# zer0main/npge

Measured on AMD Instinct MI355X. Metric: anchored+aligned Mbp/sec at 1/2/4/8 MI355X; bit-exact anchor set vs CPU, higher is better.
Workload: dtype u8

## Files before the change

### npge_amd/anchor_finder.py

```python
import ctypes

import numpy as np

from . import _capi
from .model import Block, Fragment
from .processor import Decimal, Processor, register


def seqset_for(bs):
    key = tuple((id(s), len(s.data)) for s in bs.seqs)
    cached = getattr(bs, "_npgx_seqset", None)
    if cached is not None and cached[0] == key:
        return cached[1]
    ss = _capi.SeqSet([s.data for s in bs.seqs], [s.name for s in bs.seqs])
    bs._npgx_seqset = (key, ss)
    return ss


@register
class AnchorFinder(Processor):
    name = "AnchorFinder"

    def __init__(self, bloom_params=None):
        super().__init__()
        self.add_gopt("anchor-size", "anchor size", "ANCHOR_SIZE")
        self.add_gopt("anchor-fp", "Probability of false positive in Bloom filter "
                      "(first step of AnchorFinder)", "ANCHOR_FP", Decimal)
        self.add_opt("anchor-similar", "If neighbour anchors are skipped", True)
        self.add_gopt("max-anchor-fragments", "Maximum number of anchors fragments to return",
                      "MAX_ANCHOR_FRAGMENTS")
        self.add_opt("bloom-seed", "glibc srand() seed of the Bloom hash parameters", 1)
        self.add_opt("bloom-epochs", "epochs of the one-GPU Bloom pass (0 = automatic, 1 = single pass)", 0)
        self.add_opt_rule("anchor-size > 0", lambda p: p.opt_value("anchor-size") > 0)
        self.add_opt_rule("anchor-size <= 32", lambda p: p.opt_value("anchor-size") <= 32)
        self.bloom_params = bloom_params
        self._h = None
        self._h_key = None
        self.stats = None

    def _handle(self):
        L = _capi.lib()
        key = (self.opt_value("anchor-size"), self.opt_value("anchor-fp").impl,
               bool(self.opt_value("anchor-similar")), self.opt_value("max-anchor-fragments"),
               self.opt_value("bloom-seed"), tuple(self.bloom_params or ()), self.opt_value("bloom-epochs"))
        if self._h is not None and key == self._h_key:
            return self._h
        if self._h is not None:
            L.npgx_af_free(self._h)
            self._h = None
        o = _capi.AfOptions()
        L.npgx_af_default_options(ctypes.byref(o))
        o.anchor_size, o.anchor_fp_x1e4, o.anchor_similar = key[0], key[1], int(key[2])
        o.max_anchor_fragments, o.bloom_seed = key[3], key[4] & 0xFFFFFFFF
        o.bloom_epochs = key[6]
        if self.bloom_params:
            arr = (ctypes.c_uint64 * len(self.bloom_params))(*self.bloom_params)
            o.n_bloom_params = len(self.bloom_params)
            o.bloom_params = ctypes.cast(arr, ctypes.POINTER(ctypes.c_uint64))
        h = ctypes.c_void_p()
        _capi.check(L.npgx_af_create(ctypes.byref(o), ctypes.byref(h)))
        self._h, self._h_key = h, key
        return h

    def find(self, seqset):
        L = _capi.lib()
        h = self._handle()
        _capi.check(L.npgx_af_run(h, seqset.handle))
        return self.result()

    def find_sharded(self, seqset, comm):
        L = _capi.lib()
        h = self._handle()
        rc = L.npgx_af_run_sharded(h, seqset.handle, comm.pointer())
        if rc != 0 and comm.errors:
            raise _capi.NpgxError(rc, "; ".join(comm.errors))
        _capi.check(rc)
        return self.result()

    def result(self):
        L = _capi.lib()
        h = self._h
        nb, nf = ctypes.c_int64(), ctypes.c_int64()
        _capi.check(L.npgx_af_result_counts(h, ctypes.byref(nb), ctypes.byref(nf)))
        bs = np.zeros(nb.value + 1, dtype=np.int64)
        seq = np.zeros(nf.value, dtype=np.int32)
        mn = np.zeros(nf.value, dtype=np.int64)
        mx = np.zeros(nf.value, dtype=np.int64)
        ori = np.zeros(nf.value, dtype=np.int8)
        _capi.check(L.npgx_af_result_copy(h, _capi.ptr(bs), _capi.ptr(seq), _capi.ptr(mn),
                                          _capi.ptr(mx), _capi.ptr(ori)))
        st = _capi.AfStats()
        _capi.check(L.npgx_af_stats_get(h, ctypes.byref(st)))
        self.stats = st
        return dict(block_start=bs, seq=seq, min_pos=mn, max_pos=mx, ori=ori.astype(np.int32),
                    members=st.members, bits=st.bloom_bits, hashes=st.bloom_hashes,
                    params=np.array(st.bloom_params[:st.bloom_hashes], dtype=np.uint64),
                    n_collected=st.n_collected, n_found_frags=st.n_found_frags,
                    n_windows=st.n_windows)

    def used_hashes(self):
        L = _capi.lib()
        n = ctypes.c_int64()
        _capi.check(L.npgx_af_used_hashes(self._h, None, 0, ctypes.byref(n)))
        out = np.zeros(n.value, dtype=np.uint64)
        _capi.check(L.npgx_af_used_hashes(self._h, _capi.ptr(out), n.value, ctypes.byref(n)))
        return out

    def clear_used(self):
        if self._h is not None:
            _capi.check(_capi.lib().npgx_af_clear_used(self._h))

    def kernel_times(self):
        return _capi.kernel_times(_capi.lib().npgx_af_kernel_times, self._h)

    def run_impl(self):
        bs = self.block_set()
        ss = seqset_for(bs)
        r = self.find(ss)
        b = r["block_start"]
        for i in range(len(b) - 1):
            frs = [Fragment(bs.seqs[int(r["seq"][j])], int(r["min_pos"][j]), int(r["max_pos"][j]),
                            int(r["ori"][j])) for j in range(b[i], b[i + 1])]
            bs.blocks.append(Block(frs))

    def __del__(self):
# ... 7 lines not shown
```

### npge_amd/blockset.py

```python
import ctypes

import numpy as np

from . import _capi


class BbOptions(ctypes.Structure):
    _fields_ = [("extend_length", ctypes.c_int32), ("max_iterations", ctypes.c_int32),
                ("extend_portion_x1e4", ctypes.c_int64), ("min_fragment", ctypes.c_int32),
                ("frame_length", ctypes.c_int32), ("min_end", ctypes.c_int32),
                ("min_block", ctypes.c_int32), ("max_block", ctypes.c_int32),
                ("find_subblocks", ctypes.c_int32), ("min_identity_x1e4", ctypes.c_int64),
                ("align", _capi.AlignOptions), ("max_tail", ctypes.c_int32),
                ("max_tail_to_gap_x1e4", ctypes.c_int64)]


class BbStats(ctypes.Structure):
    _fields_ = [("iterations", ctypes.c_int64), ("aligned_residues", ctypes.c_int64),
                ("align_jobs", ctypes.c_int64), ("anchor_blocks", ctypes.c_int64),
                ("stem_blocks", ctypes.c_int64), ("ms_align", ctypes.c_double),
                ("ms_host", ctypes.c_double), ("ms_stage", ctypes.c_double * 16),
                ("counters", ctypes.c_int64 * 8), ("loop", ctypes.c_int64 * 8),
                ("ms_loop", ctypes.c_double * 8), ("ms_gpu", ctypes.c_double * 12),
                ("device_iterations", ctypes.c_int64), ("device_sync_iterations", ctypes.c_int64)]
# ... 101 lines not shown
            setattr(o.align, k.replace("align_", ""), v)
        else:
            setattr(o, k, v)
    return o


class BlockSetEngine:

    def __init__(self, seqset, options=None, lender=None, **kw):
        L = _bind(_capi.lib())
        self.ss = seqset
        o = options or default_options(**kw)
        h = ctypes.c_void_p()
        if lender is None:
            _capi.check(L.npgx_blockset_create(seqset.handle, ctypes.byref(o), ctypes.byref(h)))
        else:
            _capi.check(L.npgx_blockset_create_sharing(seqset.handle, ctypes.byref(o), lender._h,
                                                       ctypes.byref(h)))
        self._lender = lender
        self._h = h

    def set_comm(self, comm):
        self._comm = comm
        _capi.check(_capi.lib().npgx_blockset_set_comm(self._h, comm.pointer() if comm else None))
        return self

    def set_blocks(self, blocks):
        L = _capi.lib()
        frs = [f for b in blocks for f in b]
        bs = np.zeros(len(blocks) + 1, dtype=np.int64)
        np.cumsum([len(b) for b in blocks], out=bs[1:])
        seq = np.array([f[0] for f in frs] or [0], dtype=np.int32)
        mn = np.array([f[1] for f in frs] or [0], dtype=np.int64)
        mx = np.array([f[2] for f in frs] or [0], dtype=np.int64)
        ori = np.array([f[3] for f in frs] or [1], dtype=np.int8)
        has_rows = any(f[4] is not None for f in frs)
        if has_rows:
            rows = "".join(f[4] or "" for f in frs).encode()
            ro = np.zeros(len(frs) + 1, dtype=np.int64)
            np.cumsum([len(f[4] or "") for f in frs], out=ro[1:])
            buf = ctypes.create_string_buffer(rows, max(len(rows), 1))
            _capi.check(L.npgx_blockset_set_blocks(self._h, len(blocks), _capi.ptr(bs), _capi.ptr(seq),
                                                   _capi.ptr(mn), _capi.ptr(mx), _capi.ptr(ori),
                                                   _capi.ptr(ro), ctypes.cast(buf, ctypes.c_void_p)))
        else:
            _capi.check(L.npgx_blockset_set_blocks(self._h, len(blocks), _capi.ptr(bs), _capi.ptr(seq),
                                                   _capi.ptr(mn), _capi.ptr(mx), _capi.ptr(ori),
                                                   None, None))
        return self

    def apply(self, processor, af=None):
        L = _capi.lib()
        afh = af._handle() if af is not None else None
        _capi.check(L.npgx_blockset_apply(self._h, processor.encode(), afh))
        return self

    def reset_loop(self):
        _capi.check(_capi.lib().npgx_blockset_reset_loop(self._h))
        return self

    def blocks(self):
        L = _capi.lib()
        nb, nf, rb = ctypes.c_int64(), ctypes.c_int64(), ctypes.c_int64()
        _capi.check(L.npgx_blockset_counts(self._h, ctypes.byref(nb), ctypes.byref(nf), ctypes.byref(rb)))
        n = max(nf.value, 1)
        bs = np.zeros(nb.value + 1, dtype=np.int64)
        seq = np.zeros(n, dtype=np.int32)
        mn = np.zeros(n, dtype=np.int64)
        mx = np.zeros(n, dtype=np.int64)
        ori = np.zeros(n, dtype=np.int8)
        ro = np.zeros(n + 1, dtype=np.int64)
        rows = ctypes.create_string_buffer(max(rb.value, 1))
        _capi.check(L.npgx_blockset_copy(self._h, _capi.ptr(bs), _capi.ptr(seq), _capi.ptr(mn),
                                         _capi.ptr(mx), _capi.ptr(ori), _capi.ptr(ro),
                                         ctypes.cast(rows, ctypes.c_void_p)))
        raw = rows.raw
        out = []
        for b in range(nb.value):
            blk = []
            for i in range(bs[b], bs[b + 1]):
                row = raw[ro[i]:ro[i + 1]].decode() if ro[i + 1] > ro[i] else None
                blk.append((int(seq[i]), int(mn[i]), int(mx[i]), int(ori[i]), row))
            out.append(blk)
        return out

    def fragments(self):
        L = _capi.lib()
        nb, nf, rb = ctypes.c_int64(), ctypes.c_int64(), ctypes.c_int64()
        _capi.check(L.npgx_blockset_counts(self._h, ctypes.byref(nb), ctypes.byref(nf), ctypes.byref(rb)))
        n = max(nf.value, 1)
        bs = np.zeros(nb.value + 1, dtype=np.int64)
        seq = np.zeros(n, dtype=np.int32)
        mn = np.zeros(n, dtype=np.int64)
        mx = np.zeros(n, dtype=np.int64)
        ori = np.zeros(n, dtype=np.int8)
        _capi.check(L.npgx_blockset_copy(self._h, _capi.ptr(bs), _capi.ptr(seq), _capi.ptr(mn),
                                         _capi.ptr(mx), _capi.ptr(ori), None, None))
        return bs, seq[:nf.value], mn[:nf.value], mx[:nf.value], ori[:nf.value]

    def conseq(self):
        L = _bind(_capi.lib())
        nb, tot = ctypes.c_int64(), ctypes.c_int64()
        _capi.check(L.npgx_blockset_conseq(self._h, None, None, ctypes.byref(nb), ctypes.byref(tot)))
        buf = ctypes.create_string_buffer(max(tot.value, 1))
        off = np.zeros(nb.value + 1, dtype=np.int64)
        _capi.check(L.npgx_blockset_conseq(self._h, ctypes.cast(buf, ctypes.c_void_p), _capi.ptr(off),
# ... 185 lines not shown
```

### npge_amd/csrc/anchor_finder.hip

```cpp
#include <rocprim/device/device_radix_sort.hpp>
#include <rocprim/device/device_scan.hpp>
#include <rocprim/device/device_select.hpp>

#include <algorithm>
#include <cmath>
#include <cstring>
#include <map>

#include <chrono>

#include "common.hpp"

namespace npgx {

std::string genome_of(const std::string& name);
uint64_t estimate_length(const npgx_seqset* s);
int64_t optimal_bits(uint64_t members, double error_prob);
int optimal_hashes(uint64_t members, uint64_t bits);
void glibc_rand(uint32_t seed, int n, uint64_t* out);

static constexpr int WG = 256;
static constexpr int MAX_KB = 32;
static constexpr int FKB = 4;

// ... 405 lines not shown
            return;
        }
        s = (s + 1) & mask;
    }
}

__global__ __launch_bounds__(WG) void k_ff_count(AfArgs a, TableArgs t, uint32_t* __restrict__ counts) {
    const Chunk c = a.chunks[blockIdx.x];
    const SeqMeta s = a.meta[c.seq];
    const int64_t p = c.pos + threadIdx.x;
    if (p + a.k > s.size) return;
    uint64_t dir;
    if (!load_window(a, s, p, dir)) return;
    const uint64_t rev = revcomp(dir, a.k);
    const uint64_t h = dir < rev ? dir : rev;
    const int64_t idx = table_find(t, h);
    if (idx >= 0) atomicAdd(&counts[idx], 1u);
}

__global__ void k_find_cut(const uint32_t* __restrict__ offsets, const uint32_t* __restrict__ counts,
                           int64_t nH, uint64_t max_frag, uint64_t* __restrict__ out ) {
    if (threadIdx.x != 0 || blockIdx.x != 0) return;
    const uint64_t total = nH ? (uint64_t)offsets[nH - 1] + counts[nH - 1] : 0;
    int64_t lo = 0, hi = nH;
    while (lo < hi) {
        int64_t mid = (lo + hi) >> 1;
        if ((uint64_t)offsets[mid] < max_frag) lo = mid + 1;
        else hi = mid;
    }
    out[0] = (uint64_t)lo;
    out[1] = lo < nH ? (uint64_t)offsets[lo] : total;
    out[2] = total;
}

__global__ __launch_bounds__(WG) void k_ff_scatter(AfArgs a, TableArgs t, const uint64_t* __restrict__ H,
                                                   uint64_t G, const uint32_t* __restrict__ offsets,
                                                   uint32_t* __restrict__ cursor, int key_bits,
                                                   uint64_t* __restrict__ cand) {
    const Chunk c = a.chunks[blockIdx.x];
    const SeqMeta s = a.meta[c.seq];
    const int64_t p = c.pos + threadIdx.x;
    if (p + a.k > s.size) return;
    uint64_t dir;
    if (!load_window(a, s, p, dir)) return;
    const uint64_t rev = revcomp(dir, a.k);
    const uint64_t h = dir < rev ? dir : rev;
    if (h > H[G - 1]) return;
    const int64_t idx = table_find(t, h);
    if (idx < 0) return;
    const uint64_t pos2 = (uint64_t)p + (h == dir ? 0ull : (uint64_t)s.size);
    const uint64_t key2 = 2ull * s.order_off + pos2;
    const uint32_t slot = offsets[idx] + atomicAdd(&cursor[idx], 1u);
    cand[slot] = ((uint64_t)idx << key_bits) | key2;
}

__global__ void k_flip_sign(uint32_t* __restrict__ v, int64_t n) {
    const int64_t i = (int64_t)blockIdx.x * blockDim.x + threadIdx.x;
    if (i < n) v[i] ^= 0x80000000u;
}

__global__ void k_local_cut(const uint32_t* __restrict__ offsets, const uint32_t* __restrict__ counts,
                            int64_t nH, uint64_t G, uint64_t* __restrict__ out) {
    if (threadIdx.x != 0 || blockIdx.x != 0) return;
    out[3] = G < (uint64_t)nH ? (uint64_t)offsets[G]
                              : (nH ? (uint64_t)offsets[nH - 1] + counts[nH - 1] : 0ull);
}

static int bits_for(uint64_t v) {
    int b = 0;
    while (b < 64 && (v > (1ull << b))) b++;
    return b;
}

}

using namespace npgx;

struct npgx_af {
    npgx_af_options opt;
    std::vector<uint64_t> explicit_params;
    int device = 0;
    hipStream_t stream = nullptr;
    std::vector<uint64_t> used;
    bool used_dirty = true;
    DevBuf<uint64_t> d_used;
    DevBuf<SeqMeta> d_meta;
    std::vector<SeqMeta> layout_meta;
    int layout_k = 0;
    int64_t layout_n = -1;
    std::vector<Chunk> layout_chunks;
    int64_t layout_c0 = -1, layout_c1 = -1, layout_local = 0;
    DevBuf<Chunk> d_chunks;
    DevBuf<uint32_t> first;
    DevBuf<uint32_t> bloom_bits;
    DevBuf<uint64_t> hraw, hsorted, huniq;
    DevBuf<uint64_t> hseg;
    DevBuf<unsigned long long> segctr;
    DevBuf<uint8_t> wmask;
    DevBuf<unsigned long long> counters;
    DevBuf<TableSlot> tslots;
    DevBuf<uint32_t> tocc;
    DevBuf<uint32_t> counts, offsets, cursor;
    DevBuf<uint32_t> counts_local, offsets_local;
    DevBuf<uint64_t> gathered;
    DevBuf<uint64_t> cut;
    DevBuf<uint64_t> cand, cand_sorted;
    DevBuf<unsigned char> temp;
    uint64_t* h_pinned = nullptr;
    PinnedBuf<uint64_t> pinned_dl;
    npgx_af_stats stats{};
    bool has_result = false;
    std::vector<int64_t> r_block_start;
    std::vector<int32_t> r_seq;
    std::vector<int64_t> r_min, r_max;
    std::vector<int8_t> r_ori;
    StageTimer timer;
    std::vector<uint64_t> host_keys, host_H;
    std::vector<size_t> h_group_key;
    bool defer_host = false;
    bool pending = false;
    bool pending_used = false;
    int64_t p_keep = 0;
    uint64_t p_G = 0;
    int p_key_bits = 0, p_k = 0;
    int32_t p_R = 0;
    std::vector<SeqMeta> p_meta;
    std::vector<int32_t> p_by_rank;
    DevBuf<int32_t> d_by_rank;
    std::vector<int32_t> d_by_rank_host;
    bool d_by_rank_valid = false;
    int64_t regroups = 0;

    void ensure_temp(size_t bytes) { temp.ensure(bytes); }
};

namespace npgx {

std::string genome_of(const std::string& name) {
    std::vector<std::string> parts;
    size_t start = 0;
    while (true) {
        size_t p = name.find('&', start);
        if (p == std::string::npos) {
            parts.push_back(name.substr(start));
            break;
        }
        parts.push_back(name.substr(start, p - start));
        start = p + 1;
    }
    if (parts.size() == 3 && (parts[2] == "c" || parts[2] == "l")) return parts[0];
    return "";
}

uint64_t estimate_length(const npgx_seqset* s) {
    std::map<std::string, uint64_t> gtl;
    uint64_t max_length = 0;
    for (int32_t i = 0; i < s->n; i++) {
        uint64_t& g = gtl[genome_of(s->names[i])];
        g += s->data[i].size();
        max_length = std::max(max_length, g);
    }
    if (gtl.size() == 1) return max_length;
    return max_length / 2 * 3;
}

static const double LN2 = 0.69314718055994530942;

int64_t optimal_bits(uint64_t members, double error_prob) {
    double v = double(members) * (-std::log(error_prob) / (LN2 * LN2)) + 0.5;
    if (!(v < 2147483647.0)) return -1;
    int r = (int)v;
    if (r % 2 == 0) r += 1;
    if (r < 1) r = 1;
    return r;
}

int optimal_hashes(uint64_t members, uint64_t bits) {
    if (members == 0) return 1;
    int r = (int)std::round(LN2 * double(bits) / double(members));
    if (r < 1) r = 1;
    return r;
}

void glibc_rand(uint32_t seed, int n, uint64_t* out) {
    std::vector<uint32_t> r(34 + 310 + (size_t)n);
    int32_t s0 = (int32_t)seed;
    if (s0 == 0) s0 = 1;
    r[0] = (uint32_t)s0;
    for (int i = 1; i < 31; i++) {
        int64_t v = (16807ll * (int32_t)r[i - 1]) % 2147483647ll;
        if (v < 0) v += 2147483647ll;
        r[i] = (uint32_t)v;
    }
    for (int i = 31; i < 34; i++) r[i] = r[i - 31];
    for (size_t i = 34; i < r.size(); i++) r[i] = r[i - 31] + r[i - 3];
    for (int i = 0; i < n; i++) out[i] = (uint64_t)(r[344 + (size_t)i] >> 1);
}

static void comm_check(int rc, const char* what) {
    if (rc != 0) throw Error(NPGX_ERR_ARG, std::string("collective callback failed: ") + what);
}

static void af_group_host(npgx_af* af, const std::vector<uint64_t>& keys, const std::vector<uint64_t>& Hh,
                          int key_bits, int32_t R, const SeqMeta* meta, const int32_t* by_rank, int k,
                          bool add_used);
static void af_materialize(npgx_af* af);
static void af_pending_used(npgx_af* af);

static void af_run(npgx_af* af, const npgx_seqset* ss, const npgx_comm* comm) {
    static const bool hdbg = getenv("NPGX_AF_DEBUG") != nullptr;
    const auto th0 = std::chrono::steady_clock::now();
    auto hms = [&]() { return std::chrono::duration<double, std::milli>(std::chrono::steady_clock::now() - th0).count(); };
    double h_prep = 0, h_dl = 0;
    NPGX_REQUIRE(ss->device == af->device, NPGX_ERR_ARG, "sequence set and finder on different devices");
    NPGX_HIP(hipSetDevice(af->device));
    hipStream_t st = af->stream;
    const int k = af->opt.anchor_size;
    if (af->pending) {
        if (af->pending_used) af_pending_used(af);
        af->pending = false;
    }
    af->timer.reset();
    af->has_result = false;
    npgx_af_stats& S = af->stats;
    memset(&S, 0, sizeof(S));

    uint64_t members = estimate_length(ss);
    if (k * 2 < 64) members = std::min<uint64_t>(members, 1ull << (2 * k));
    const double fp = double(af->opt.anchor_fp_x1e4) / 10000.0;
    const int64_t m = optimal_bits(members, fp);
    NPGX_REQUIRE(m > 0, NPGX_ERR_RANGE, "Bloom filter size overflows the reference's int");
    const int kb = optimal_hashes(members, (uint64_t)m);
    NPGX_REQUIRE(kb <= MAX_KB, NPGX_ERR_RANGE, "too many Bloom hash functions");
    AfArgs A;
    memset(&A, 0, sizeof(A));
    if (!af->explicit_params.empty()) {
        NPGX_REQUIRE((int)af->explicit_params.size() >= kb, NPGX_ERR_ARG,
                     "explicit Bloom parameter vector shorter than the hash count");
        for (int i = 0; i < kb; i++) A.params[i] = af->explicit_params[i];
    } else {
        glibc_rand(af->opt.bloom_seed, kb, A.params);
    }
    S.members = (int64_t)members;
    S.bloom_bits = m;
    S.bloom_hashes = kb;
    for (int i = 0; i < kb; i++) S.bloom_params[i] = A.params[i];

    int32_t R = 0;
    while (R < ss->n && (int64_t)ss->data[ss->by_rank[R]].size() >= k) R++;
    std::vector<SeqMeta> meta(R > 0 ? R : 1);
    uint64_t order = 0;
    int64_t n_windows = 0;
    for (int32_t r = 0; r < R; r++) {
        const int64_t size = (int64_t)ss->data[ss->by_rank[r]].size();
        meta[r] = SeqMeta{size, ss->word_off[r], ss->n_off[r], order};
        order += (uint64_t)size;
        n_windows += size - k + 1;
    }
    const bool same_layout = af->layout_k == k && af->layout_meta.size() == meta.size() &&
                             memcmp(af->layout_meta.data(), meta.data(), meta.size() * sizeof(SeqMeta)) == 0;
    std::vector<Chunk>& chunks = af->layout_chunks;
    if (!same_layout) {
        chunks.clear();
        for (int32_t r = 0; r < R; r++)
            for (int64_t p = 0; p < meta[r].size - k + 1; p += WG) chunks.push_back(Chunk{r, 0, p});
    }
    static const uint64_t max_bases = [] {
        const char* e = getenv("NPGX_AF_MAX_BASES");
        const uint64_t v = e ? strtoull(e, nullptr, 10) : 0;
        return v > 0 && v < 0xFFFFFFFEull ? v : 0xFFFFFFFEull;
    }();
    NPGX_REQUIRE(order < max_bases, NPGX_ERR_RANGE, "more than 2^32-2 bases in one run (32-bit window orders)");
    S.n_windows = n_windows;
    S.n_used = (int64_t)af->used.size();
// ... 209 lines not shown
                NPGX_HIP(hipMemcpyAsync(af->hraw.p + hp[0], &h0, 8, hipMemcpyHostToDevice, st));
                NPGX_HIP(hipMemcpyAsync(af->counters.p, &n1, 8, hipMemcpyHostToDevice, st));
                NPGX_HIP(stream_wait(st));
            }
        }
    }
    NPGX_HIP(hipMemcpyAsync(hp, af->counters.p, 8, hipMemcpyDeviceToHost, st));
    NPGX_HIP(stream_wait(st));
    const int64_t n_raw = (int64_t)hp[0];
    S.n_collected_raw = n_raw;

    const unsigned h_end_bit = (unsigned)std::min(64, 2 * k);
    auto sort_unique = [&](const uint64_t* in, int64_t n) -> int64_t {
        if (n <= 0) return 0;
        af->hsorted.ensure((size_t)n);
        af->huniq.ensure((size_t)n);
        size_t b1 = 0, b2 = 0;
        NPGX_HIP(rocprim::radix_sort_keys(nullptr, b1, in, af->hsorted.p, (size_t)n, 0u, h_end_bit, st));
        NPGX_HIP(rocprim::unique(nullptr, b2, af->hsorted.p, af->huniq.p, af->counters.p + 1,
                                 (size_t)n, rocprim::equal_to<uint64_t>(), st));
        af->ensure_temp(std::max(b1, b2));
        size_t t = af->timer.begin("sort_unique_H", st, n * 8.0 * 4, n);
        NPGX_HIP(rocprim::radix_sort_keys(af->temp.p, b1, in, af->hsorted.p, (size_t)n, 0u, h_end_bit, st));
        NPGX_HIP(rocprim::unique(af->temp.p, b2, af->hsorted.p, af->huniq.p, af->counters.p + 1,
                                 (size_t)n, rocprim::equal_to<uint64_t>(), st));
        af->timer.end(t, st);
        NPGX_HIP(hipMemcpyAsync(hp, af->counters.p + 1, 8, hipMemcpyDeviceToHost, st));
        NPGX_HIP(stream_wait(st));
        return (int64_t)hp[0];
    };
    std::vector<int64_t> rc(world);
    auto gather_u64 = [&](const uint64_t* src, int64_t n, const char* what) -> int64_t {
        comm_check(comm->allgather_i64(comm->user, n, rc.data()), what);
        int64_t tot = 0;
        for (int64_t v : rc) tot += v;
        af->gathered.grow((size_t)std::max<int64_t>(tot, 1));
        NPGX_HIP(stream_wait(st));
        if (tot > 0) comm_check(comm->allgatherv_u64(comm->user, src, rc.data(), af->gathered.p), what);
        return tot;
    };
    int64_t nH = sort_unique(af->hraw.p, n_raw);
    if (comm) {
        const int64_t tot = gather_u64(af->huniq.p, nH, "allgatherv(collected hashes)");
        nH = sort_unique(af->gathered.p, tot);
    }
    S.n_collected = nH;

    std::vector<uint64_t>& keys = af->host_keys;
    std::vector<uint64_t>& Hh = af->host_H;
    keys.clear();
    Hh.clear();
    uint64_t G = 0;
    int key_bits = bits_for(2ull * order);
    if (nH > 0) {
        uint64_t cap = 1024;
        static const uint64_t spf = getenv("NPGX_AF_TABLE_SLOTS") ? std::max(2, atoi(getenv("NPGX_AF_TABLE_SLOTS"))) : 4;
        while (cap < spf * (uint64_t)nH) cap <<= 1;
        NPGX_REQUIRE(cap <= (1ull << 31), NPGX_ERR_RANGE, "hash set too large");
        int log2cap = 0;
        while ((1ull << log2cap) < cap) log2cap++;
        af->tslots.ensure(cap);
        af->tocc.ensure((size_t)(cap + 31) / 32);
        TableArgs T{af->tslots.p, af->tocc.p, (uint32_t)(cap - 1), 64 - log2cap};
        ti = af->timer.begin("table_insert", st, nH * 8.0 + nH * 12.0, nH);
        af->counts.ensure((size_t)nH);
        af->offsets.ensure((size_t)nH);
        af->cursor.ensure((size_t)nH);
        fills.add(af->tslots.p, (int64_t)(cap * sizeof(TableSlot)), 0xFFFFFFFFu);
        fills.add(af->tocc.p, (int64_t)(cap + 31) / 32 * 4, 0u);
        fills.add(af->counts.p, nH * 4, 0u);
        fills.add(af->cursor.p, nH * 4, 0u);
        fills.launch(st);
        NPGX_HIP(hipGetLastError());
        hipLaunchKernelGGL(k_table_insert, dim3((unsigned)((nH + 255) / 256)), dim3(256), 0, st,
                           af->huniq.p, nH, af->tslots.p, af->tocc.p, (uint32_t)(cap - 1),
                           64 - log2cap);
        NPGX_HIP(hipGetLastError());
        af->timer.end(ti, st);

        ti = af->timer.begin("ff_count", st, local_windows * (0.375 + 12.0), local_windows);
        if (run_local) hipLaunchKernelGGL(k_ff_count, grid, block, 0, st, A, T, af->counts.p);
        NPGX_HIP(hipGetLastError());
        af->timer.end(ti, st);
        if (comm) {
            af->counts_local.ensure((size_t)nH);
            af->offsets_local.ensure((size_t)nH);
            NPGX_HIP(hipMemcpyAsync(af->counts_local.p, af->counts.p, (size_t)nH * 4,
                                    hipMemcpyDeviceToDevice, st));
            NPGX_HIP(stream_wait(st));
            comm_check(comm->allreduce_i32(comm->user, (int32_t*)af->counts.p, nH, NPGX_OP_SUM),
                       "allreduce(counts, SUM)");
        }
        size_t b3 = 0;
        NPGX_HIP(rocprim::exclusive_scan(nullptr, b3, af->counts.p, af->offsets.p, 0u, (size_t)nH,
                                         rocprim::plus<uint32_t>(), st));
        af->ensure_temp(b3);
        ti = af->timer.begin("scan_cut", st, nH * 8.0, nH);
        NPGX_HIP(rocprim::exclusive_scan(af->temp.p, b3, af->counts.p, af->offsets.p, 0u,
                                         (size_t)nH, rocprim::plus<uint32_t>(), st));
        af->cut.ensure(4);
        hipLaunchKernelGGL(k_find_cut, dim3(1), dim3(64), 0, st, af->offsets.p, af->counts.p, nH,
                           (uint64_t)af->opt.max_anchor_fragments, af->cut.p);
        NPGX_HIP(hipGetLastError());
        af->timer.end(ti, st);
        NPGX_HIP(hipMemcpyAsync(hp, af->cut.p, 3 * 8, hipMemcpyDeviceToHost, st));
        NPGX_HIP(stream_wait(st));
        G = hp[0];
        const uint64_t C = hp[1];
        S.n_found_frags = (int64_t)hp[2];
        S.n_kept_groups = (int64_t)G;
        if (G > 0 && C > 0) {
            const int idx_bits = bits_for(G);
            NPGX_REQUIRE(idx_bits + key_bits <= 64, NPGX_ERR_RANGE,
                         "FoundFragment sort key does not fit 64 bits");
            uint64_t C_local = C;
            const uint32_t* scatter_off = af->offsets.p;
            if (comm) {
                NPGX_HIP(rocprim::exclusive_scan(af->temp.p, b3, af->counts_local.p, af->offsets_local.p,
                                                 0u, (size_t)nH, rocprim::plus<uint32_t>(), st));
                hipLaunchKernelGGL(k_local_cut, dim3(1), dim3(64), 0, st, af->offsets_local.p,
                                   af->counts_local.p, nH, G, af->cut.p);
                NPGX_HIP(hipGetLastError());
                NPGX_HIP(hipMemcpyAsync(hp, af->cut.p + 3, 8, hipMemcpyDeviceToHost, st));
                NPGX_HIP(stream_wait(st));
                C_local = hp[0];
                scatter_off = af->offsets_local.p;
            }
            af->cand.ensure(std::max<uint64_t>(C_local, 1));
            af->cand_sorted.ensure(C);
            ti = af->timer.begin("ff_scatter", st, local_windows * 0.375 + C_local * 24.0, local_windows);
            if (run_local && C_local > 0)
                hipLaunchKernelGGL(k_ff_scatter, grid, block, 0, st, A, T, af->huniq.p, G, scatter_off,
                                   af->cursor.p, key_bits, af->cand.p);
            NPGX_HIP(hipGetLastError());
            af->timer.end(ti, st);
            const uint64_t* sort_in = af->cand.p;
            if (comm) {
                const int64_t tot = gather_u64(af->cand.p, (int64_t)C_local, "allgatherv(FoundFragments)");
                NPGX_REQUIRE((uint64_t)tot == C, NPGX_ERR_STATE, "sharded FoundFragment count mismatch");
                sort_in = af->gathered.p;
            }
            size_t b4 = 0;
            const unsigned end_bit = (unsigned)(idx_bits + key_bits);
            NPGX_HIP(rocprim::radix_sort_keys(nullptr, b4, sort_in, af->cand_sorted.p, (size_t)C, 0u,
                                              end_bit, st));
            af->ensure_temp(b4);
            ti = af->timer.begin("ff_sort", st, C * 32.0, (int64_t)C);
            NPGX_HIP(rocprim::radix_sort_keys(af->temp.p, b4, sort_in, af->cand_sorted.p, (size_t)C,
                                              0u, end_bit, st));
            af->timer.end(ti, st);
            const uint64_t keep = std::min<uint64_t>(C, (uint64_t)af->opt.max_anchor_fragments);
            if (af->defer_host && !comm && keep > 0) {
                af->pending = true;
                af->pending_used = true;
                af->p_keep = (int64_t)keep;
                af->p_G = G;
                af->p_key_bits = key_bits;
                af->p_k = k;
                af->p_R = R;
                af->p_meta.assign(meta.begin(), meta.begin() + R);
                af->p_by_rank.assign(ss->by_rank.begin(), ss->by_rank.begin() + R);
                if (!af->d_by_rank_valid || af->d_by_rank_host != af->p_by_rank) {
                    af->d_by_rank_valid = false;
                    af->d_by_rank.ensure((size_t)std::max<int32_t>(R, 1));
                    int32_t* hb = (int32_t*)af->pinned_dl.ensure((size_t)R / 2 + 2);
                    memcpy(hb, af->p_by_rank.data(), (size_t)R * 4);
                    NPGX_HIP(hipMemcpyAsync(af->d_by_rank.p, hb, (size_t)R * 4, hipMemcpyHostToDevice, st));
                    af->d_by_rank_host = af->p_by_rank;
                    af->d_by_rank_valid = true;
                }
                NPGX_HIP(stream_wait(st));
                S.n_blocks = S.n_fragments = -1;
                af->has_result = true;
                return;
            }
            keys.resize(keep);
            Hh.resize(G);
            af->pinned_dl.ensure((keep + G) * 8);
            uint64_t* pk = af->pinned_dl.p;
            NPGX_HIP(hipMemcpyAsync(pk, af->cand_sorted.p, keep * 8, hipMemcpyDeviceToHost, st));
            NPGX_HIP(hipMemcpyAsync(pk + keep, af->huniq.p, G * 8, hipMemcpyDeviceToHost, st));
            NPGX_HIP(stream_wait(st));
            memcpy(keys.data(), pk, keep * 8);
            memcpy(Hh.data(), pk + keep, G * 8);
        }
    }

    h_dl = hms();
    af_group_host(af, keys, Hh, key_bits, R, meta.data(), ss->by_rank.data(), k, true);
    if (hdbg)
        fprintf(stderr, "af host: prep %.3f ms, results downloaded at %.3f ms, grouping %.3f ms (%zu keys, %lld blocks)\n",
                h_prep, h_dl, hms() - h_dl, keys.size(), (long long)S.n_blocks);
}

static void af_group_host(npgx_af* af, const std::vector<uint64_t>& keys, const std::vector<uint64_t>& Hh,
                          int key_bits, int32_t R, const SeqMeta* meta, const int32_t* by_rank, int k,
                          bool add_used) {
    npgx_af_stats& S = af->stats;
    std::vector<uint64_t> prefix2(R);
    for (int32_t r = 0; r < R; r++) prefix2[r] = 2ull * meta[r].order_off;
    const uint64_t key_mask = key_bits >= 64 ? ~0ull : ((1ull << key_bits) - 1);
    const bool sort_used = !af->used.empty();
    const size_t nk = keys.size();
    std::vector<size_t>& gk = af->h_group_key;
    gk.clear();
    af->r_block_start.clear();
    int64_t nout = 0;
    bool first_group = true;
    for (size_t i = 0; i < nk;) {
        const uint64_t idx = keys[i] >> key_bits;
        size_t j = i + 1;
        while (j < nk && (keys[j] >> key_bits) == idx) j++;
        if (!first_group && add_used) af->used.push_back(Hh[idx]);
        first_group = false;
        if (j - i >= 2) {
            af->r_block_start.push_back(nout);
            gk.push_back(i);
            nout += (int64_t)(j - i);
        }
        i = j;
    }
    af->r_block_start.push_back(nout);
    af->r_seq.resize((size_t)nout);
    af->r_min.resize((size_t)nout);
    af->r_max.resize((size_t)nout);
    af->r_ori.resize((size_t)nout);
    const size_t ng = gk.size(), per = 256;
    heavy_for((ng + per - 1) / per, nout * 16, [&](size_t t) {
// ... 14 lines not shown
            af->r_ori[(size_t)o] = direct ? 1 : -1;
        }
      }
    });
    if (sort_used) std::sort(af->used.begin(), af->used.end());
    if (af->used.size() != (size_t)S.n_used) af->used_dirty = true;
    S.n_blocks = (int64_t)af->r_block_start.size() - 1;
    S.n_fragments = (int64_t)af->r_seq.size();
    S.n_used = (int64_t)af->used.size();
    af->has_result = true;
}

static void af_download_pending(npgx_af* af) {
    hipStream_t st = af->stream;
    NPGX_HIP(hipSetDevice(af->device));
    std::vector<uint64_t>& keys = af->host_keys;
    std::vector<uint64_t>& Hh = af->host_H;
    keys.resize((size_t)af->p_keep);
    Hh.resize((size_t)af->p_G);
    af->pinned_dl.ensure((size_t)(af->p_keep + af->p_G) * 8 + 8);
    uint64_t* pk = af->pinned_dl.p;
    if (af->p_keep) NPGX_HIP(hipMemcpyAsync(pk, af->cand_sorted.p, (size_t)af->p_keep * 8, hipMemcpyDeviceToHost, st));
    if (af->p_G) NPGX_HIP(hipMemcpyAsync(pk + af->p_keep, af->huniq.p, (size_t)af->p_G * 8, hipMemcpyDeviceToHost, st));
    NPGX_HIP(stream_wait(st));
    memcpy(keys.data(), pk, (size_t)af->p_keep * 8);
    memcpy(Hh.data(), pk + af->p_keep, (size_t)af->p_G * 8);
}

static void af_materialize(npgx_af* af) {
    if (!af->pending) return;
    af->pending = false;
    af_download_pending(af);
    af->regroups++;
    af_group_host(af, af->host_keys, af->host_H, af->p_key_bits, af->p_R, af->p_meta.data(),
                  af->p_by_rank.data(), af->p_k, af->pending_used);
}

static void af_pending_used(npgx_af* af) {
    af_download_pending(af);
    const std::vector<uint64_t>& keys = af->host_keys;
    const std::vector<uint64_t>& Hh = af->host_H;
    const int key_bits = af->p_key_bits;
    const bool sort_used = !af->used.empty();
    const size_t nk = keys.size(), n0 = af->used.size();
    for (size_t i = 1; i < nk; i++) {
        const uint64_t idx = keys[i] >> key_bits;
        if (idx != (keys[i - 1] >> key_bits)) af->used.push_back(Hh[idx]);
    }
    if (sort_used) std::sort(af->used.begin(), af->used.end());
    if (af->used.size() != n0) af->used_dirty = true;
    af->pending_used = false;
}

void af_set_defer(npgx_af* af, bool on) { af->defer_host = on; }

bool af_device_keys(npgx_af* af, AfDevKeys* o) {
    if (!af->pending) return false;
    o->keys = af->cand_sorted.p;
    o->keep = af->p_keep;
    o->key_bits = af->p_key_bits;
    o->k = af->p_k;
    o->R = af->p_R;
    o->meta = af->d_meta.p;
    o->by_rank = af->d_by_rank.p;
    return true;
}

}

extern "C" {

void npgx_af_default_options(npgx_af_options* o) {
    if (!o) return;
    memset(o, 0, sizeof(*o));
    o->anchor_size = 20;
    o->anchor_similar = 1;
    o->anchor_fp_x1e4 = 1000;
    o->max_anchor_fragments = 100000;
    o->bloom_seed = 1;
}

int npgx_af_create(const npgx_af_options* o, npgx_af** out) {
    return guard([&] {
        NPGX_REQUIRE(o && out, NPGX_ERR_ARG, "null argument");
        NPGX_REQUIRE(o->anchor_size > 0, NPGX_ERR_ARG, "Option rule failed: anchor-size > 0");
        NPGX_REQUIRE(o->anchor_size <= 32, NPGX_ERR_ARG, "Option rule failed: anchor-size <= 32");
        NPGX_REQUIRE(o->anchor_fp_x1e4 > 0 && o->anchor_fp_x1e4 < 10000, NPGX_ERR_ARG,
                     "anchor-fp must be in (0, 1)");
        NPGX_REQUIRE(o->max_anchor_fragments >= 0, NPGX_ERR_ARG, "max-anchor-fragments < 0");
        NPGX_REQUIRE(o->n_bloom_params >= 0 && o->n_bloom_params <= MAX_KB, NPGX_ERR_ARG,
                     "n_bloom_params out of range");
        NPGX_REQUIRE(o->bloom_epochs >= 0, NPGX_ERR_ARG, "bloom_epochs < 0");
        int dev = current_device_checked();
        auto* af = new npgx_af;
        af->opt = *o;
        af->opt.bloom_params = nullptr;
        if (o->n_bloom_params > 0)
            af->explicit_params.assign(o->bloom_params, o->bloom_params + o->n_bloom_params);
        af->device = dev;
        if (hipStreamCreateWithFlags(&af->stream, hipStreamNonBlocking) != hipSuccess ||
            hipHostMalloc((void**)&af->h_pinned, 64) != hipSuccess) {
            delete af;
            throw Error(NPGX_ERR_HIP, "stream / pinned allocation failed");
        }
        *out = af;
    });
}

int npgx_af_run(npgx_af* af, const npgx_seqset* s) {
    return guard([&] {
        NPGX_REQUIRE(af && s, NPGX_ERR_ARG, "null argument");
        af_run(af, s, nullptr);
    });
}

int npgx_af_run_sharded(npgx_af* af, const npgx_seqset* s, const npgx_comm* comm) {
    return guard([&] {
        NPGX_REQUIRE(af && s && comm, NPGX_ERR_ARG, "null argument");
        NPGX_REQUIRE(comm->world >= 1 && comm->rank >= 0 && comm->rank < comm->world, NPGX_ERR_ARG,
                     "bad rank / world");
        NPGX_REQUIRE(comm->allreduce_i32 && comm->allgather_i64 && comm->allgatherv_u64, NPGX_ERR_ARG,
                     "missing collective callback");
        af_run(af, s, comm->world > 1 ? comm : nullptr);
    });
}

int npgx_af_stats_get(const npgx_af* af, npgx_af_stats* out) {
    return guard([&] {
        NPGX_REQUIRE(af && out, NPGX_ERR_ARG, "null argument");
        const int64_t regroups = af->regroups;
        af_materialize(const_cast<npgx_af*>(af));
        *out = af->stats;
        out->host_regroups = regroups;
    });
}

int npgx_af_result_counts(const npgx_af* af, int64_t* nb, int64_t* nf) {
    return guard([&] {
        NPGX_REQUIRE(af && nb && nf, NPGX_ERR_ARG, "null argument");
        NPGX_REQUIRE(af->has_result, NPGX_ERR_STATE, "no AnchorFinder result yet");
        af_materialize(const_cast<npgx_af*>(af));
        *nb = (int64_t)af->r_block_start.size() - 1;
        *nf = (int64_t)af->r_seq.size();
    });
}

int npgx_af_result_copy(const npgx_af* af, int64_t* block_start, int32_t* seq, int64_t* min_pos,
                        int64_t* max_pos, int8_t* ori) {
    return guard([&] {
        NPGX_REQUIRE(af, NPGX_ERR_ARG, "null argument");
        NPGX_REQUIRE(af->has_result, NPGX_ERR_STATE, "no AnchorFinder result yet");
        af_materialize(const_cast<npgx_af*>(af));
        const size_t nf = af->r_seq.size();
        if (block_start) memcpy(block_start, af->r_block_start.data(), af->r_block_start.size() * 8);
        if (seq) memcpy(seq, af->r_seq.data(), nf * 4);
        if (min_pos) memcpy(min_pos, af->r_min.data(), nf * 8);
        if (max_pos) memcpy(max_pos, af->r_max.data(), nf * 8);
        if (ori) memcpy(ori, af->r_ori.data(), nf);
    });
}

int npgx_af_used_hashes(const npgx_af* af, uint64_t* out, int64_t cap, int64_t* n) {
    return guard([&] {
        NPGX_REQUIRE(af && n, NPGX_ERR_ARG, "null argument");
        af_materialize(const_cast<npgx_af*>(af));
        *n = (int64_t)af->used.size();
        if (out) memcpy(out, af->used.data(), (size_t)std::min<int64_t>(cap, *n) * 8);
    });
}

int npgx_af_clear_used(npgx_af* af) {
    return guard([&] {
        NPGX_REQUIRE(af, NPGX_ERR_ARG, "null argument");
        af->used.clear();
        af->pending_used = false;
        af->used_dirty = true;
    });
}

int npgx_af_kernel_times(const npgx_af* af, npgx_kernel_time* out, int32_t cap, int32_t* n) {
    return guard([&] {
        NPGX_REQUIRE(af && n && (out || cap == 0), NPGX_ERR_ARG, "null argument");
        af->timer.copy_out(out, cap, n);
    });
// ... 12 lines not shown
```

Measured before the change: 2687.

## Collect capped FoundFragments in one pass and defer total-count computation

```diff
diff --git a/npge_amd/anchor_finder.py b/npge_amd/anchor_finder.py
--- a/npge_amd/anchor_finder.py
+++ b/npge_amd/anchor_finder.py
@@ -36,6 +36,7 @@
         self.bloom_params = bloom_params
         self._h = None
         self._h_key = None
+        self._last_set = None
         self.stats = None
 
     def _handle(self):
@@ -65,12 +66,14 @@
     def find(self, seqset):
         L = _capi.lib()
         h = self._handle()
+        self._last_set = seqset
         _capi.check(L.npgx_af_run(h, seqset.handle))
         return self.result()
 
     def find_sharded(self, seqset, comm):
         L = _capi.lib()
         h = self._handle()
+        self._last_set = seqset
         rc = L.npgx_af_run_sharded(h, seqset.handle, comm.pointer())
         if rc != 0 and comm.errors:
             raise _capi.NpgxError(rc, "; ".join(comm.errors))
diff --git a/npge_amd/blockset.py b/npge_amd/blockset.py
--- a/npge_amd/blockset.py
+++ b/npge_amd/blockset.py
@@ -177,6 +177,8 @@
     def apply(self, processor, af=None):
         L = _capi.lib()
         afh = af._handle() if af is not None else None
+        if af is not None:
+            af._last_set = self.ss
         _capi.check(L.npgx_blockset_apply(self._h, processor.encode(), afh))
         return self
 
diff --git a/npge_amd/csrc/anchor_finder.hip b/npge_amd/csrc/anchor_finder.hip
--- a/npge_amd/csrc/anchor_finder.hip
+++ b/npge_amd/csrc/anchor_finder.hip
@@ -481,6 +481,31 @@
     const uint64_t key2 = 2ull * s.order_off + pos2;
     const uint32_t slot = offsets[idx] + atomicAdd(&cursor[idx], 1u);
     cand[slot] = ((uint64_t)idx << key_bits) | key2;
+}
+
+__global__ __launch_bounds__(WG) void k_ff_collect(AfArgs a, TableArgs t, const uint64_t* __restrict__ H, int64_t L,
+                                                   int key_bits, uint64_t* __restrict__ out,
+                                                   unsigned long long* __restrict__ n_out) {
+    const Chunk c = a.chunks[blockIdx.x];
+    const SeqMeta s = a.meta[c.seq];
+    const int64_t p = c.pos + threadIdx.x;
+    bool col = false;
+    uint64_t key = 0;
+    uint64_t dir;
+    if (p + a.k <= s.size && load_window(a, s, p, dir)) {
+        const uint64_t rev = revcomp(dir, a.k);
+        const uint64_t h = dir < rev ? dir : rev;
+        if (h <= H[L - 1]) {
+            const int64_t idx = table_find(t, h);
+            if (idx >= 0) {
+                const uint64_t pos2 = (uint64_t)p + (h == dir ? 0ull : (uint64_t)s.size);
+                key = ((uint64_t)idx << key_bits) | (2ull * s.order_off + pos2);
+                col = true;
+            }
+        }
+    }
+    const int64_t seg = (int64_t)blockIdx.x % a.nseg;
+    wg_append(col, key, out + seg * a.seg_cap, n_out + seg * 16);
 }
 
 __global__ void k_flip_sign(uint32_t* __restrict__ v, int64_t n) {
@@ -559,6 +584,9 @@
     std::vector<int32_t> d_by_rank_host;
     bool d_by_rank_valid = false;
     int64_t regroups = 0;
+    bool found_pending = false;
+    AfArgs f_A{};
+    int64_t f_nchunks = 0, f_windows = 0, f_nH = 0;
 
     void ensure_temp(size_t bytes) { temp.ensure(bytes); }
 };
@@ -630,11 +658,63 @@
     if (rc != 0) throw Error(NPGX_ERR_ARG, std::string("collective callback failed: ") + what);
 }
 
+static TableArgs af_table_prepare(npgx_af* af, int64_t n, Fills& fills) {
+    uint64_t cap = 1024;
+    static const uint64_t spf = getenv("NPGX_AF_TABLE_SLOTS") ? std::max(2, atoi(getenv("NPGX_AF_TABLE_SLOTS"))) : 4;
+    while (cap < spf * (uint64_t)n) cap <<= 1;
+    NPGX_REQUIRE(cap <= (1ull << 31), NPGX_ERR_RANGE, "hash set too large");
+    int log2cap = 0;
+    while ((1ull << log2cap) < cap) log2cap++;
+    af->tslots.ensure(cap);
+    af->tocc.ensure((size_t)(cap + 31) / 32);
+    fills.add(af->tslots.p, (int64_t)(cap * sizeof(TableSlot)), 0xFFFFFFFFu);
+    fills.add(af->tocc.p, (int64_t)(cap + 31) / 32 * 4, 0u);
+    return TableArgs{af->tslots.p, af->tocc.p, (uint32_t)(cap - 1), 64 - log2cap};
+}
+
+static void af_table_insert(npgx_af* af, const TableArgs& T, int64_t n, hipStream_t st) {
+    hipLaunchKernelGGL(k_table_insert, dim3((unsigned)((n + 255) / 256)), dim3(256), 0, st, af->huniq.p, n,
+                       af->tslots.p, af->tocc.p, T.mask, T.shift);
+    NPGX_HIP(hipGetLastError());
+}
+
+static void af_found_total_enqueue(npgx_af* af, const AfArgs& A, int64_t nchunks, int64_t windows, int64_t nH) {
+    hipStream_t st = af->stream;
+    Fills fills;
+    const TableArgs T = af_table_prepare(af, nH, fills);
+    af->counts.ensure((size_t)nH);
+    af->offsets.ensure((size_t)nH);
+    size_t ti = af->timer.begin("table_insert", st, nH * 8.0 + nH * 12.0, nH);
+    fills.add(af->counts.p, nH * 4, 0u);
+    fills.launch(st);
+    NPGX_HIP(hipGetLastError());
+    af_table_insert(af, T, nH, st);
+    af->timer.end(ti, st);
+    ti = af->timer.begin("ff_count", st, windows * (0.375 + 12.0), windows);
+    hipLaunchKernelGGL(k_ff_count, dim3((unsigned)nchunks), dim3(WG), 0, st, A, T, af->counts.p);
+    NPGX_HIP(hipGetLastError());
+    af->timer.end(ti, st);
+    size_t b3 = 0;
+    NPGX_HIP(rocprim::exclusive_scan(nullptr, b3, af->counts.p, af->offsets.p, 0u, (size_t)nH,
+                                     rocprim::plus<uint32_t>(), st));
+    af->ensure_temp(b3);
+    ti = af->timer.begin("scan_cut", st, nH * 8.0, nH);
+    NPGX_HIP(rocprim::exclusive_scan(af->temp.p, b3, af->counts.p, af->offsets.p, 0u, (size_t)nH,
+                                     rocprim::plus<uint32_t>(), st));
+    af->cut.ensure(4);
+    hipLaunchKernelGGL(k_find_cut, dim3(1), dim3(64), 0, st, af->offsets.p, af->counts.p, nH,
+                       (uint64_t)af->opt.max_anchor_fragments, af->cut.p);
+    NPGX_HIP(hipGetLastError());
+    af->timer.end(ti, st);
+    NPGX_HIP(hipMemcpyAsync(af->h_pinned + 4, af->cut.p, 3 * 8, hipMemcpyDeviceToHost, st));
+}
+
 static void af_group_host(npgx_af* af, const std::vector<uint64_t>& keys, const std::vector<uint64_t>& Hh,
                           int key_bits, int32_t R, const SeqMeta* meta, const int32_t* by_rank, int k,
                           bool add_used);
 static void af_materialize(npgx_af* af);
 static void af_pending_used(npgx_af* af);
+static void af_found_pending(npgx_af* af);
 
 static void af_run(npgx_af* af, const npgx_seqset* ss, const npgx_comm* comm) {
     static const bool hdbg = getenv("NPGX_AF_DEBUG") != nullptr;
@@ -649,6 +729,7 @@
         if (af->pending_used) af_pending_used(af);
         af->pending = false;
     }
+    af->found_pending = false;
     af->timer.reset();
     af->has_result = false;
     npgx_af_stats& S = af->stats;
@@ -964,45 +1045,116 @@
     Hh.clear();
     uint64_t G = 0;
     int key_bits = bits_for(2ull * order);
-    if (nH > 0) {
-        uint64_t cap = 1024;
-        static const uint64_t spf = getenv("NPGX_AF_TABLE_SLOTS") ? std::max(2, atoi(getenv("NPGX_AF_TABLE_SLOTS"))) : 4;
-        while (cap < spf * (uint64_t)nH) cap <<= 1;
-        NPGX_REQUIRE(cap <= (1ull << 31), NPGX_ERR_RANGE, "hash set too large");
-        int log2cap = 0;
-        while ((1ull << log2cap) < cap) log2cap++;
-        af->tslots.ensure(cap);
-        af->tocc.ensure((size_t)(cap + 31) / 32);
-        TableArgs T{af->tslots.p, af->tocc.p, (uint32_t)(cap - 1), 64 - log2cap};
-        ti = af->timer.begin("table_insert", st, nH * 8.0 + nH * 12.0, nH);
+    if (nH > 0 && !comm) {
+        const uint64_t max_frag = (uint64_t)af->opt.max_anchor_fragments;
+        const int64_t L = (int64_t)std::min<uint64_t>((uint64_t)nH, max_frag + 1);
+        const int idx_bits = bits_for((uint64_t)L);
+        NPGX_REQUIRE(idx_bits + key_bits <= 64, NPGX_ERR_RANGE, "FoundFragment sort key does not fit 64 bits");
+        const TableArgs T = af_table_prepare(af, L, fills);
+        ti = af->timer.begin("table_insert", st, L * 8.0 + L * 12.0, L);
+        fills.add(af->segctr.p, (int64_t)A.nseg * 16 * 8, 0u);
+        fills.launch(st);
+        NPGX_HIP(hipGetLastError());
+        af_table_insert(af, T, L, st);
+        af->timer.end(ti, st);
+        ti = af->timer.begin("ff_collect", st, local_windows * 0.375, local_windows);
+        hipLaunchKernelGGL(k_ff_collect, grid, block, 0, st, A, T, af->huniq.p, L, key_bits, af->hseg.p,
+                           af->segctr.p);
+        NPGX_HIP(hipGetLastError());
+        hipLaunchKernelGGL(k_seg_compact, dim3((unsigned)A.nseg), dim3(256), 0, st, af->hseg.p, af->segctr.p,
+                           A.nseg, A.seg_cap, af->hraw.p, af->counters.p + 2);
+        NPGX_HIP(hipGetLastError());
+        af->timer.end(ti, st);
+        NPGX_HIP(hipMemcpyAsync(hp, af->counters.p + 2, 8, hipMemcpyDeviceToHost, st));
+        NPGX_HIP(stream_wait(st));
+        const uint64_t n_keys = hp[0];
+        const uint64_t keep = std::min<uint64_t>(n_keys, max_frag);
+        if (keep > 0) {
+            af->cand_sorted.ensure(n_keys);
+            size_t b4 = 0;
+            const unsigned end_bit = (unsigned)(idx_bits + key_bits);
+            NPGX_HIP(rocprim::radix_sort_keys(nullptr, b4, af->hraw.p, af->cand_sorted.p, (size_t)n_keys, 0u,
+                                              end_bit, st));
+            af->ensure_temp(b4);
+            ti = af->timer.begin("ff_sort", st, n_keys * 32.0, (int64_t)n_keys);
+            NPGX_HIP(rocprim::radix_sort_keys(af->temp.p, b4, af->hraw.p, af->cand_sorted.p, (size_t)n_keys, 0u,
+                                              end_bit, st));
+            af->timer.end(ti, st);
+            NPGX_HIP(hipMemcpyAsync(hp + 1, af->cand_sorted.p + (keep - 1), 8, hipMemcpyDeviceToHost, st));
+        }
+        if (af->defer_host && keep > 0) {
+            af->p_by_rank.assign(ss->by_rank.begin(), ss->by_rank.begin() + R);
+            if (!af->d_by_rank_valid || af->d_by_rank_host != af->p_by_rank) {
+                af->d_by_rank_valid = false;
+                af->d_by_rank.ensure((size_t)std::max<int32_t>(R, 1));
+                int32_t* hb = (int32_t*)af->pinned_dl.ensure((size_t)R / 2 + 2);
+                memcpy(hb, af->p_by_rank.data(), (size_t)R * 4);
+                NPGX_HIP(hipMemcpyAsync(af->d_by_rank.p, hb, (size_t)R * 4, hipMemcpyHostToDevice, st));
+                af->d_by_rank_host = af->p_by_rank;
+                af->d_by_rank_valid = true;
+            }
+            NPGX_HIP(stream_wait(st));
+            G = (hp[1] >> key_bits) + 1;
+            af->pending = true;
+            af->pending_used = true;
+            af->p_keep = (int64_t)keep;
+            af->p_G = G;
+            af->p_key_bits = key_bits;
+            af->p_k = k;
+            af->p_R = R;
+            af->p_meta.assign(meta.begin(), meta.begin() + R);
+            S.n_kept_groups = (int64_t)G;
+            S.n_blocks = S.n_fragments = -1;
+            S.n_found_frags = -1;
+            af->found_pending = true;
+            af->f_A = A;
+            af->f_nchunks = nchunks;
+            af->f_windows = local_windows;
+            af->f_nH = nH;
+            af->has_result = true;
+            return;
+        }
+        af_found_total_enqueue(af, A, nchunks, local_windows, nH);
+        if (keep > 0) {
+            NPGX_HIP(stream_wait(st));
+            G = (hp[1] >> key_bits) + 1;
+            keys.resize(keep);
+            Hh.resize(G);
+            af->pinned_dl.ensure((keep + G) * 8);
+            uint64_t* pk = af->pinned_dl.p;
+            NPGX_HIP(hipMemcpyAsync(pk, af->cand_sorted.p, keep * 8, hipMemcpyDeviceToHost, st));
+            NPGX_HIP(hipMemcpyAsync(pk + keep, af->huniq.p, G * 8, hipMemcpyDeviceToHost, st));
+            NPGX_HIP(stream_wait(st));
+            memcpy(keys.data(), pk, keep * 8);
+            memcpy(Hh.data(), pk + keep, G * 8);
+        } else {
+            NPGX_HIP(stream_wait(st));
+        }
+        S.n_found_frags = (int64_t)hp[6];
+        S.n_kept_groups = (int64_t)G;
+    } else if (nH > 0) {
+        const TableArgs T = af_table_prepare(af, nH, fills);
         af->counts.ensure((size_t)nH);
         af->offsets.ensure((size_t)nH);
         af->cursor.ensure((size_t)nH);
-        fills.add(af->tslots.p, (int64_t)(cap * sizeof(TableSlot)), 0xFFFFFFFFu);
-        fills.add(af->tocc.p, (int64_t)(cap + 31) / 32 * 4, 0u);
+        ti = af->timer.begin("table_insert", st, nH * 8.0 + nH * 12.0, nH);
         fills.add(af->counts.p, nH * 4, 0u);
         fills.add(af->cursor.p, nH * 4, 0u);
         fills.launch(st);
         NPGX_HIP(hipGetLastError());
-        hipLaunchKernelGGL(k_table_insert, dim3((unsigned)((nH + 255) / 256)), dim3(256), 0, st,
-                           af->huniq.p, nH, af->tslots.p, af->tocc.p, (uint32_t)(cap - 1),
-                           64 - log2cap);
-        NPGX_HIP(hipGetLastError());
+        af_table_insert(af, T, nH, st);
         af->timer.end(ti, st);
 
         ti = af->timer.begin("ff_count", st, local_windows * (0.375 + 12.0), local_windows);
         if (run_local) hipLaunchKernelGGL(k_ff_count, grid, block, 0, st, A, T, af->counts.p);
         NPGX_HIP(hipGetLastError());
         af->timer.end(ti, st);
-        if (comm) {
-            af->counts_local.ensure((size_t)nH);
-            af->offsets_local.ensure((size_t)nH);
-            NPGX_HIP(hipMemcpyAsync(af->counts_local.p, af->counts.p, (size_t)nH * 4,
-                                    hipMemcpyDeviceToDevice, st));
-            NPGX_HIP(stream_wait(st));
-            comm_check(comm->allreduce_i32(comm->user, (int32_t*)af->counts.p, nH, NPGX_OP_SUM),
-                       "allreduce(counts, SUM)");
-        }
+        af->counts_local.ensure((size_t)nH);
+        af->offsets_local.ensure((size_t)nH);
+        NPGX_HIP(hipMemcpyAsync(af->counts_local.p, af->counts.p, (size_t)nH * 4, hipMemcpyDeviceToDevice, st));
+        NPGX_HIP(stream_wait(st));
+        comm_check(comm->allreduce_i32(comm->user, (int32_t*)af->counts.p, nH, NPGX_OP_SUM),
+                   "allreduce(counts, SUM)");
         size_t b3 = 0;
         NPGX_HIP(rocprim::exclusive_scan(nullptr, b3, af->counts.p, af->offsets.p, 0u, (size_t)nH,
                                          rocprim::plus<uint32_t>(), st));
@@ -1025,33 +1177,25 @@
             const int idx_bits = bits_for(G);
             NPGX_REQUIRE(idx_bits + key_bits <= 64, NPGX_ERR_RANGE,
                          "FoundFragment sort key does not fit 64 bits");
-            uint64_t C_local = C;
-            const uint32_t* scatter_off = af->offsets.p;
-            if (comm) {
-                NPGX_HIP(rocprim::exclusive_scan(af->temp.p, b3, af->counts_local.p, af->offsets_local.p,
-                                                 0u, (size_t)nH, rocprim::plus<uint32_t>(), st));
-                hipLaunchKernelGGL(k_local_cut, dim3(1), dim3(64), 0, st, af->offsets_local.p,
-                                   af->counts_local.p, nH, G, af->cut.p);
-                NPGX_HIP(hipGetLastError());
-                NPGX_HIP(hipMemcpyAsync(hp, af->cut.p + 3, 8, hipMemcpyDeviceToHost, st));
-                NPGX_HIP(stream_wait(st));
-                C_local = hp[0];
-                scatter_off = af->offsets_local.p;
-            }
+            NPGX_HIP(rocprim::exclusive_scan(af->temp.p, b3, af->counts_local.p, af->offsets_local.p,
+                                             0u, (size_t)nH, rocprim::plus<uint32_t>(), st));
+            hipLaunchKernelGGL(k_local_cut, dim3(1), dim3(64), 0, st, af->offsets_local.p,
+                               af->counts_local.p, nH, G, af->cut.p);
+            NPGX_HIP(hipGetLastError());
+            NPGX_HIP(hipMemcpyAsync(hp, af->cut.p + 3, 8, hipMemcpyDeviceToHost, st));
+            NPGX_HIP(stream_wait(st));
+            const uint64_t C_local = hp[0];
             af->cand.ensure(std::max<uint64_t>(C_local, 1));
             af->cand_sorted.ensure(C);
             ti = af->timer.begin("ff_scatter", st, local_windows * 0.375 + C_local * 24.0, local_windows);
             if (run_local && C_local > 0)
-                hipLaunchKernelGGL(k_ff_scatter, grid, block, 0, st, A, T, af->huniq.p, G, scatter_off,
+                hipLaunchKernelGGL(k_ff_scatter, grid, block, 0, st, A, T, af->huniq.p, G, af->offsets_local.p,
                                    af->cursor.p, key_bits, af->cand.p);
             NPGX_HIP(hipGetLastError());
             af->timer.end(ti, st);
-            const uint64_t* sort_in = af->cand.p;
-            if (comm) {
-                const int64_t tot = gather_u64(af->cand.p, (int64_t)C_local, "allgatherv(FoundFragments)");
-                NPGX_REQUIRE((uint64_t)tot == C, NPGX_ERR_STATE, "sharded FoundFragment count mismatch");
-                sort_in = af->gathered.p;
-            }
+            const int64_t tot = gather_u64(af->cand.p, (int64_t)C_local, "allgatherv(FoundFragments)");
+            NPGX_REQUIRE((uint64_t)tot == C, NPGX_ERR_STATE, "sharded FoundFragment count mismatch");
+            const uint64_t* sort_in = af->gathered.p;
             size_t b4 = 0;
             const unsigned end_bit = (unsigned)(idx_bits + key_bits);
             NPGX_HIP(rocprim::radix_sort_keys(nullptr, b4, sort_in, af->cand_sorted.p, (size_t)C, 0u,
@@ -1062,30 +1206,6 @@
                                               0u, end_bit, st));
             af->timer.end(ti, st);
             const uint64_t keep = std::min<uint64_t>(C, (uint64_t)af->opt.max_anchor_fragments);
-            if (af->defer_host && !comm && keep > 0) {
-                af->pending = true;
-                af->pending_used = true;
-                af->p_keep = (int64_t)keep;
-                af->p_G = G;
-                af->p_key_bits = key_bits;
-                af->p_k = k;
-                af->p_R = R;
-                af->p_meta.assign(meta.begin(), meta.begin() + R);
-                af->p_by_rank.assign(ss->by_rank.begin(), ss->by_rank.begin() + R);
-                if (!af->d_by_rank_valid || af->d_by_rank_host != af->p_by_rank) {
-                    af->d_by_rank_valid = false;
-                    af->d_by_rank.ensure((size_t)std::max<int32_t>(R, 1));
-                    int32_t* hb = (int32_t*)af->pinned_dl.ensure((size_t)R / 2 + 2);
-                    memcpy(hb, af->p_by_rank.data(), (size_t)R * 4);
-                    NPGX_HIP(hipMemcpyAsync(af->d_by_rank.p, hb, (size_t)R * 4, hipMemcpyHostToDevice, st));
-                    af->d_by_rank_host = af->p_by_rank;
-                    af->d_by_rank_valid = true;
-                }
-                NPGX_HIP(stream_wait(st));
-                S.n_blocks = S.n_fragments = -1;
-                af->has_result = true;
-                return;
-            }
             keys.resize(keep);
             Hh.resize(G);
             af->pinned_dl.ensure((keep + G) * 8);
@@ -1206,6 +1326,15 @@
     af->pending_used = false;
 }
 
+static void af_found_pending(npgx_af* af) {
+    if (!af->found_pending) return;
+    NPGX_HIP(hipSetDevice(af->device));
+    af_found_total_enqueue(af, af->f_A, af->f_nchunks, af->f_windows, af->f_nH);
+    NPGX_HIP(stream_wait(af->stream));
+    af->stats.n_found_frags = (int64_t)af->h_pinned[6];
+    af->found_pending = false;
+}
+
 void af_set_defer(npgx_af* af, bool on) { af->defer_host = on; }
 
 bool af_device_keys(npgx_af* af, AfDevKeys* o) {
@@ -1284,6 +1413,7 @@
         NPGX_REQUIRE(af && out, NPGX_ERR_ARG, "null argument");
         const int64_t regroups = af->regroups;
         af_materialize(const_cast<npgx_af*>(af));
+        af_found_pending(const_cast<npgx_af*>(af));
         *out = af->stats;
         out->host_regroups = regroups;
     });
```

After: 2751, median of 6. 2.4% higher.
